# kazuto1011/dusty-gan

Hardware: AMD Instinct MI355X
Metric: G+D train images/sec on 64x1024 LiDAR (steps/sec beside it) (higher is better)
Workload: dtype bf16

## Files before the change

dusty_gan_amd/_lib.py:

```python
import ctypes as C
import os
import subprocess

_HERE = os.path.dirname(os.path.abspath(__file__))
CSRC = os.path.join(_HERE, "csrc")
LIB_PATH = os.path.join(CSRC, "libdustygan_hip.so")
if os.environ.get("DUSTY_GAN_LIB_DIAG"):
    _d = os.environ["DUSTY_GAN_LIB_DIAG"]
    LIB_PATH = os.path.join(CSRC, "libdustygan_hip_diag%s.so" % ("" if _d == "1" else _d))

DG_OK, DG_EINVAL, DG_EUNSUPPORTED, DG_EHIP = 0, 1, 2, 3
DG_F32, DG_BF16 = 0, 1
DG_BF16X2 = 2
MODE_S2, MODE_UP, MODE_GEMM = 0, 1, 2
EPI_LINEAR, EPI_LRELU, EPI_MASK = 0, 1, 2
DG_FORCE_FP32X3 = 0x100
POLICY_BITS = {"brightness": 1, "saturation": 2, "contrast": 4, "translation": 8, "cutout": 16}

_ERR = {1: "DG_EINVAL (bad argument)", 2: "DG_EUNSUPPORTED (shape not supported by the requested kernel)",
        3: "DG_EHIP (HIP runtime error)"}


class DgError(RuntimeError):
    pass
# ... 36 lines not shown
                ("eps", C.c_float), ("ilo", C.c_int), ("ihi", C.c_int), ("n", C.c_long), ("out", C.c_void_p),
                ("out_bf16", C.c_void_p), ("B", C.c_int), ("H", C.c_int), ("W", C.c_int), ("uf", C.c_void_p),
                ("qi", C.c_void_p)]


class DgWgrad(C.Structure):
    _fields_ = [
        ("wmode", C.c_int), ("ring", C.c_int),
        ("B", C.c_int), ("Hc", C.c_int), ("Wc", C.c_int),
        ("Ci", C.c_int), ("Co", C.c_int),
        ("a", C.c_void_p), ("a_sb", C.c_long), ("a_sp", C.c_long), ("a_sc", C.c_long),
        ("g", C.c_void_p), ("g_sb", C.c_long), ("g_sp", C.c_long), ("g_sc", C.c_long),
        ("dw", C.c_void_p), ("scale", C.c_float), ("rowscale", C.c_void_p),
        ("a_dtype", C.c_int), ("g_dtype", C.c_int),
        ("ws", C.c_void_p), ("g_mod", C.c_int),
    ]


XSUM_PARTS = 8


class DgFetch(C.Structure):
    _fields_ = [("pol", C.c_void_p), ("mask", C.c_void_p), ("pool_ctr", C.c_void_p), ("npool", C.c_int),
                ("min_depth", C.c_float), ("max_depth", C.c_float), ("drop_const", C.c_float), ("B", C.c_int), ("HW", C.c_long),
                ("out", C.c_void_p), ("parts", C.c_void_p)]


class DgAugSet(C.Structure):
    _fields_ = [("x", C.c_void_p), ("xsum", C.c_void_p), ("xsum_parts", C.c_int), ("u_b", C.c_void_p), ("u_c", C.c_void_p), ("t_h", C.c_void_p),
                ("t_w", C.c_void_p), ("o_x", C.c_void_p), ("o_y", C.c_void_p)]


class DgOptSeg(C.Structure):
    _fields_ = [("off", C.c_longlong), ("numel", C.c_longlong), ("part", C.c_void_p), ("splits", C.c_int), ("accumulate", C.c_int),
                ("kind", C.c_int), ("ci", C.c_int), ("co", C.c_int), ("shadow_t", C.c_void_p), ("ws_src", C.c_void_p),
                ("ws_coef", C.c_void_p), ("ws_stride", C.c_longlong), ("ws_n", C.c_int), ("ws_bf16", C.c_int),
                ("ws_scale", C.c_float), ("first_block", C.c_int)]


OPT_MAX_SEG = 20


class DgWgradPlan(C.Structure):
    _fields_ = [("variant", C.c_int), ("splits", C.c_int), ("ws_floats", C.c_long), ("tap_pairs", C.c_int)]


class DgWgradReduce(C.Structure):
    _fields_ = [("ws", C.c_void_p), ("dw", C.c_void_p), ("numel", C.c_long), ("splits", C.c_int), ("accumulate", C.c_int)]


class DgConvPlan(C.Structure):
    _fields_ = [("family", C.c_int), ("bm", C.c_int), ("bn", C.c_int), ("tiles", C.c_int), ("workgroups", C.c_int),
                ("tiles_per_wg", C.c_int), ("thin_mfma", C.c_int), ("mask_bits", C.c_int), ("dbias_rows", C.c_int),
                ("sum_parts", C.c_int)]


_P, _I, _L, _F, _D, _U64 = C.c_void_p, C.c_int, C.c_long, C.c_float, C.c_double, C.c_uint64

PROTOTYPES = {
    "dg_conv": [C.POINTER(DgConv), _I, _P],
    "dg_conv_ex": [C.POINTER(DgConv), _I, _I, _P],
    "dg_conv_plan": [C.POINTER(DgConv), _I, _I, C.POINTER(DgConvPlan)],
    "dg_conv_mfma_supported": [C.POINTER(DgConv)],
    "dg_conv_kernel_choice": [C.POINTER(DgConv)],
    "dg_wgrad": [C.POINTER(DgWgrad), _I, _I, _P],
    "dg_wgrad_plan": [C.POINTER(DgWgrad), _I, _I, C.POINTER(DgWgradPlan)],
    "dg_wgrad_group": [C.POINTER(DgWgrad), _I, _I, _I, _P],
    "dg_wgrad_group_plan": [C.POINTER(DgWgrad), _I, _I, _I, C.POINTER(DgWgradPlan)],
    "dg_wgrad_reduce": [C.POINTER(DgWgradReduce), _I, _P],
    "dg_wgrad_mfma_supported": [C.POINTER(DgWgrad)],
    "dg_wgrad_kernel_choice": [C.POINTER(DgWgrad)],
    "dg_wgrad_kernel_variant": [C.POINTER(DgWgrad), _I],
    "dg_wgrad_has_sample_map": [C.POINTER(DgWgrad), _I],
    "dg_blur_fwd": [_P, _P, _I, _I, _I, _I, _I, _P],
    "dg_blur_fwd_mean": [_P, _P, _I, _I, _I, _I, _I, _P, _I, _P, _P],
    "dg_blur_bwd": [_P, _I, _P, _I, _I, _I, _I, _P],
    "dg_blur_bwd_r1": [_P, _I, _P, _F, _P, _I, _I, _I, _I, _P],
    "dg_blur_r1_tangent": [_P, _I, _P, _F, _P, _P, _I, _I, _I, _I, _I, _P],
    "dg_final_fwd": [_P, _I, _P, _P, _F, _I, _L, _P, _P],
    "dg_final_fwd_acc": [_P, _I, _P, _P, _F, _I, _L, _P, _P],
    "dg_final_bwd_data": [_P, _I, _P, _P, _P, _F, _I, _L, _I, _P, _P, _P],
    "dg_batch_wsum": [_P, _I, _P, _F, _I, _L, _P, _P],
    "dg_head_post_fwd": [_P, _P, _P, _I, _I, _F, _F, _I, _L, _P, _P, _P],
    "dg_head_post_fwd_sum": [_P, _P, _P, _I, _I, _F, _F, _I, _L, _P, _P, _P, _P],
    "dg_head_post_bwd": [_P, _P, _P, _P, _P, _I, _F, _F, _I, _L, _F, _F, _P, _P, _P, _I, _P, _P],
    "dg_logistic_noise": [_P, _P, _F, _L, _P, _P],
    "dg_diffaug_fwd": [_P, _P, _P, _P, _P, _P, _P, _I, _I, _I, _I, _P, _P, _P],
    "dg_diffaug_bwd": [_P, _P, _P, _P, _P, _P, _P, _I, _I, _I, _I, _P, _P, _P],
    "dg_diffaug_fwd_acc": [_P, _P, _P, _P, _P, _P, _P, _I, _I, _I, _I, _P, _P, _P],
    "dg_diffaug_fwd_pre": [_P, _P, _P, _P, _P, _P, _P, _I, _I, _I, _I, _P, _P, _P],
    "dg_diffaug_bwd_acc": [_P, _P, _P, _P, _P, _P, _P, _I, _I, _I, _I, _P, _P, _P],
    "dg_diffaug_blur_fwd": [C.POINTER(DgAugSet), _I, _I, _I, _I, _I, _I, _P, _I, _P],
    "dg_blur_bwd_augsum": [_P, _I, _P, _P, _P, _P, _I, _P, _I, _I, _I, _I, _P],
    "dg_diffaug_bwd_pre": [_P, _P, _P, _P, _P, _P, _P, _I, _I, _I, _I, _P, _P, _P],
    "dg_head_post_bwd_aug": [_P, _P, _P, _P, _P, _P, _P, _P, _P, _P, _P, _I, _P, _I, _F, _F, _I, _I, _I, _F, _F, _P, _P, _P,
                             _I, _P, _P],
    "dg_fetch_reals_pool_sum": [_P, _P, _P, _I, _F, _F, _F, _I, _L, _P, _P, _P],
    "dg_nsgan_d": [_P, _P, _I, _F, _P, _P, _P, _P],
    "dg_nsgan_g": [_P, _I, _F, _P, _P, _P],
    "dg_nsgan_d_step": [_P, _P, _I, _F, _P, _P, _P, _P, _P, _P],
    "dg_nsgan_g_step": [_P, _I, _F, _P, _P, _P],
    "dg_gan_d_step": [_I, _F, _P, _P, _I, _F, _P, _P, _P, _P, _P, _P],
    "dg_gan_g_step": [_I, _P, _P, _I, _F, _P, _P, _P],
    "dg_final_gan_bwd": [_I, _I, _F, _P, _P, _I, _F, _I, _P, _P, _P, _P, _P, _P, _I, _P, _F, _L, _I, _P, _P, _P, _P, _P],
    "dg_det_arena": [_P, _L, _P],
    "dg_mean_acc": [_P, _I, _P, _P],
    "dg_fetch_reals": [_P, _P, _F, _F, _F, _L, _P, _P],
# ... 329 lines not shown
```

dusty_gan_amd/csrc/conv_mfma_pp.hip:

```cpp
#include "conv_mfma_persist_impl.h"

#include <type_traits>

namespace pp {

using persist::Geo;
using persist::Tile;

typedef __attribute__((ext_vector_type(4))) float f32x4_t;

#define PP_WAIT(vm) asm volatile("s_waitcnt vmcnt(%0) lgkmcnt(0)" ::"n"(vm) : "memory")

constexpr int NHT = 256;
struct HTab { unsigned long long e[NHT]; };

__device__ __forceinline__ unsigned long long pp_stamp() {
  unsigned long long t;
  __builtin_amdgcn_sched_barrier(0);
  asm volatile("s_memtime %0\n\ts_waitcnt lgkmcnt(0)" : "=s"(t)::"memory");
  __builtin_amdgcn_sched_barrier(0);
  return t;
}

template <int CTRL>
__device__ __forceinline__ float row_add(float v) {
  const int s = __builtin_amdgcn_update_dpp(0, __builtin_bit_cast(int, v), CTRL, 0xf, 0xf, false);
  return v + __builtin_bit_cast(float, s);
}

template <int BN, int MODE, bool MASK, bool DUAL = false, bool BITS = false, bool X2 = false>
__global__ __launch_bounds__(512, 2) void conv_pp_kernel(ConvP p, Geo g, HTab ht) {
  static_assert(MASK || !BITS, "BITS: a flavour of the EPI_MASK epilogue");
  static_assert(!X2 || !BITS, "X2: mask source = the saved activation's hi half");
  static_assert(!DUAL || (MODE == MODE_UP && BN == 128), "DUAL: both column parities of a 64-channel MODE_UP layer");
  constexpr int NCH = DUAL ? BN / 2 : BN;
  constexpr int BM = 256, NWV = 8, WN = 2;
  constexpr int SB = 128;
  constexpr int WC = BN / WN;
  constexpr int TM = 4, TN = WC / 16;
  constexpr int CPL = 4 * TN;
  constexpr int IMG_ROWS = 264;
  constexpr int AIMG = IMG_ROWS * SB;
  constexpr int BT = BN * SB;
  constexpr int PSTAGE = AIMG + 2 * BT;
  constexpr int NPS = 2;
  constexpr int IA = 4, IB = BN / 8 / NWV;
  constexpr int NST = TM * CPL * 2 / 16;
  constexpr int NDB = 512;
  constexpr int NPAIR = MODE == MODE_S2 ? 2 : 1;
  constexpr bool STRIP = BN == 128 && !X2;
  constexpr int SCR = STRIP ? 16 * WC * 2 : 0;
  constexpr int NDBR = 4;
  constexpr int NDBX = MASK ? (NDBR - 2) * NDB : 0;
  constexpr int DBW = DUAL ? NWV : NWV / WN;
  constexpr int LDS_HT = NPS * PSTAGE + 3 * NDB * 4 + NDBX * 4 + NWV * SCR;
  static_assert(IB >= 1 && LDS_HT <= 160 * 1024, "LDS");
  __shared__ __attribute__((aligned(1024))) unsigned char lds[LDS_HT];
#ifdef DG_PP_DIAG
  constexpr int dbg = DG_PP_DIAG;
#else
  constexpr int dbg = 0;
#endif

  const int G = gridDim.x;
  const int q8 = G >> 3, r8 = G & 7, xcd = blockIdx.x & 7;
  const int gi0 = xcd < r8 ? xcd * (q8 + 1) : r8 * (q8 + 1) + (xcd - r8) * q8;
  const int nwx = q8 + (xcd < r8 ? 1 : 0);
// ... 2 lines not shown
  const int xe = (gi0 + nwx) * tq + (gi0 + nwx < tr ? gi0 + nwx : tr);
  const int t0 = xs + (int)(blockIdx.x >> 3);
  const int tcount = t0 < xe ? (xe - t0 + nwx - 1) / nwx : 0;
  if (tcount == 0) {
    if (MASK && p.dbias && p.dbias_part)
      for (int n = threadIdx.x; n < p.N; n += 64 * NWV) p.dbias_part[(long)blockIdx.x * p.N + n] = 0.f;
    return;
  }

  const unsigned long long tk0 = (dbg & 8) ? pp_stamp() : 0ull;
  const unsigned long long tr0 = (dbg & 8) ? __builtin_amdgcn_s_memrealtime() : 0ull;
  const int tid = threadIdx.x;
  const int wave = __builtin_amdgcn_readfirstlane(tid >> 6), lane = tid & 63;
  const int KC = p.K / 64;
  const int Ws = MODE == MODE_S2 ? 2 * p.Wc : p.Wc, cmul = MODE == MODE_S2 ? 2 : 1;
  const int Wo = MODE == MODE_S2 ? p.Wc : 2 * p.Wc;
  const int rows = MODE == MODE_S2 ? p.Hc : 2 * p.Hc;
  const int tiles_n = g.tiles_n, tiles_x = g.tiles_x;

  auto tile_at = [&](int t) {
    Tile r;
    int mt = t / tiles_n;
    r.nt = t % tiles_n;
    r.px = 0;
    r.xt = mt % tiles_x; mt /= tiles_x;
    if (MODE == MODE_UP && !DUAL) { r.px = mt & 1; mt >>= 1; }
    r.Y = mt % rows; r.bt = mt / rows;
    r.nt = __builtin_amdgcn_readfirstlane(r.nt); r.xt = __builtin_amdgcn_readfirstlane(r.xt);
    r.px = __builtin_amdgcn_readfirstlane(r.px); r.Y = __builtin_amdgcn_readfirstlane(r.Y);
    r.bt = __builtin_amdgcn_readfirstlane(r.bt);
    return r;
  };
  const Tile first = tile_at(t0);
  Tile dstep;
  {
    int r = nwx;
    dstep.nt = r % tiles_n; r /= tiles_n;
    dstep.xt = r % tiles_x; r /= tiles_x;
    dstep.px = 0;
    if (MODE == MODE_UP && !DUAL) { dstep.px = r & 1; r >>= 1; }
    dstep.Y = r % rows; dstep.bt = r / rows;
    dstep.nt = __builtin_amdgcn_readfirstlane(dstep.nt); dstep.xt = __builtin_amdgcn_readfirstlane(dstep.xt);
    dstep.px = __builtin_amdgcn_readfirstlane(dstep.px); dstep.Y = __builtin_amdgcn_readfirstlane(dstep.Y);
    dstep.bt = __builtin_amdgcn_readfirstlane(dstep.bt);
  }
  auto tile_next = [&](Tile& t) __attribute__((always_inline)) {
    int c;
    t.nt += dstep.nt; c = t.nt >= tiles_n; if (c) t.nt -= tiles_n;
    t.xt += dstep.xt + c; c = t.xt >= tiles_x; if (c) t.xt -= tiles_x;
    if (MODE == MODE_UP && !DUAL) { t.px += dstep.px + c; c = t.px >> 1; t.px &= 1; }
    t.Y += dstep.Y + c; c = t.Y >= rows; if (c) t.Y -= rows;
    t.bt += dstep.bt + c;
  };

  const bf16* in = (const bf16*)p.in;
  const bf16* w = (const bf16*)p.w;
  const int lrow = lane >> 3, pos = lane & 7;
  auto swzA = [](int row) { return ((row >> 1) & 3) << 1; };
  auto swzB = [](int row) { return ((row >> 1) & 1) | (((row / CPL) & 3) << 1); };

  unsigned voffA[NPAIR][IA + 1], voffB[IB];
  int colA[IA + 1];
  unsigned sampA[IA + 1];
  {
    const int pitch = g.SW + (DUAL ? 2 : 1);
#pragma unroll
    for (int u = 0; u <= IA; ++u) {
      const int m = (u < IA ? (wave + NWV * u) : 32) * 8 + lrow;
      int seg = m / pitch, c = m - seg * pitch;
      if (seg >= g.NSB) { seg = 0; c = 0; }
      colA[u] = cmul * c;
      sampA[u] = (unsigned)(seg * (int)p.in_sb * 2 + (pos ^ swzA(m)) * 16);
    }
  }
#pragma unroll
  for (int u = 0; u < IB; ++u) {
    const int row = (wave + NWV * u) * 8 + lrow;
    voffB[u] = (unsigned)((DUAL ? row & 63 : row) * (int)p.w_sn * 2 + (pos ^ swzB(row)) * 16);
  }
  const unsigned dst_wave = (unsigned)wave * 1024u;

  const int wm = wave >> 1, wn = wave & 1;
  const int a16 = lane & 15, g4 = lane >> 4;
  const unsigned lds0 = (unsigned)(size_t)(__attribute__((address_space(3))) unsigned char*)lds;
  unsigned pbase[2];
  {
    const int rowbase = ((wm * 64) >> g.lsw) * (g.SW + (DUAL ? 2 : 1)) + ((wm * 64) & (g.SW - 1));
#pragma unroll
    for (int t = 0; t < 2; ++t) {
      const int r = rowbase + a16 + t + (DUAL ? wn : 0);
      pbase[t] = (unsigned)(r * SB + ((g4 ^ swzA(r)) << 4));
    }
  }
  const unsigned wrow = (unsigned)(wn * WC + (a16 >> 2) * CPL + (a16 & 3));
  const unsigned wbase = (unsigned)(AIMG + wrow * SB + ((g4 ^ (((a16 >> 1) & 1) | ((a16 >> 2) << 1))) << 4));

  float* s_rs = (float*)(lds + NPS * PSTAGE);
  float* s_bias = s_rs + NDB;
  float* s_db = s_bias + NDB;
  const unsigned srs0 = lds0 + NPS * PSTAGE, sbias0 = srs0 + NDB * 4, sdb0 = sbias0 + NDB * 4;
  const bool want_db = MASK && p.dbias != nullptr;
  const bool db_rows = MASK && DBW * p.N <= NDBR * NDB;
  const unsigned sdbw0 = db_rows ? sbias0 + (unsigned)((DUAL ? wave : wave / WN) * p.N) * 4u : sdb0;
  for (int i = tid; i < NDB; i += 64 * NWV) {
    s_bias[i] = (!MASK && p.bias && i < p.N) ? p.bias[i % p.bias_mod] * (p.epi == EPI_LRELU ? SQRT2 : 1.f) : 0.f;
    s_db[i] = 0.f;
    s_rs[i] = (p.rowscale && i < p.B) ? p.rowscale[i] : 1.f;
  }
  if (MASK)
    for (int i = tid; i < NDBX; i += 64 * NWV) s_db[NDB + i] = 0.f;
  __syncthreads();
  const unsigned long long tk1 = (dbg & 8) ? pp_stamp() : 0ull;

  f32x4_t acc[TM][TN];
  auto zero_acc = [&]() __attribute__((always_inline)) {
#pragma unroll
    for (int i = 0; i < TM; ++i)
#pragma unroll
      for (int j = 0; j < TN; ++j) acc[i][j] = f32x4_t{0.f, 0.f, 0.f, 0.f};
  };
  zero_acc();
  i32x4 fp[2][TM], fw[2][TN];

  bf16* out = (bf16*)p.out;
  const unsigned lane_c0 = (unsigned)((DUAL ? 0 : wn * WC) + g4 * CPL);
  const unsigned lane_coff = X2 ? lane_c0 * 2 + ((lane_c0 >> 6) << 7) : lane_c0 * 2;
  const unsigned par_off = DUAL ? (unsigned)(wn * (int)p.out_sp * 2) : 0u;
  const long px_b = (long)(MODE == MODE_S2 ? 1 : 2) * p.out_sp * 2;
  unsigned pix_off;
  {
    const int trow = wm * 64 + a16;
    const int sb = trow >> g.lsw, x = trow & (g.SW - 1);
    pix_off = (unsigned)((sb * (int)p.out_sb + (MODE == MODE_S2 ? x : 2 * x) * (int)p.out_sp) * 2) + lane_coff + par_off;
  }
  constexpr int CH = WC / 8;
  constexpr int RPB = 64 / CH;
  constexpr int NRD = 16 / RPB;
  static_assert(NRD == NST / TM, "strip geometry");
  auto swzS = [](int px) { return CH == 8 ? (px & 7) : ((px >> 1) & 3); };
  const unsigned scr0 = lds0 + NPS * PSTAGE + 3 * NDB * 4 + NDBX * 4 + (unsigned)wave * SCR;
  const unsigned scr_w = scr0 + (unsigned)(a16 * (CH * 16) + (((g4 * NRD) ^ swzS(a16)) << 4));
  unsigned scr_r, st_off;
  {
    const int pr = lane / CH, c = lane % CH;
    scr_r = scr0 + (unsigned)(pr * (CH * 16) + ((c ^ swzS(pr)) << 4));
    const int trow = wm * 64 + pr;
    const int sb = trow >> g.lsw, x = trow & (g.SW - 1);
    st_off = (unsigned)((sb * (int)p.out_sb + (MODE == MODE_S2 ? x : 2 * x) * (int)p.out_sp) * 2 + c * 16) +
             (DUAL ? par_off : (unsigned)((wn * WC) * 2));
  }
  static_assert(NRD == 1 || RPB * CH * 16 == 1024, "strip read offset");
  auto tile_off = [&](const Tile& t) __attribute__((always_inline)) -> long {
    const int n0 = t.xt * BM;
    return (long)(t.bt * g.NSB) * p.out_sb + ((long)t.Y * Wo + (MODE == MODE_S2 ? n0 : 2 * n0 + t.px)) * p.out_sp +
           t.nt * NCH * (X2 ? 2 : 1);
  };
  i32x4 axr[(MASK && !BITS) ? NST : 1];
  unsigned mbits[BITS ? TM : 1];
  const unsigned pix_off_m = pix_off >> 4;
  auto load_aux = [&](const Tile& t) __attribute__((always_inline)) {
    if constexpr (BITS) {
      const char* mb = (const char*)p.mask_in + (tile_off(t) >> 3);
#pragma unroll
      for (int i = 0; i < TM; ++i) {
        const char* src = mb + (long)i * px_b;
        if (CPL == 16) asm volatile("global_load_ushort %0, %1, %2" : "=v"(mbits[i]) : "v"(pix_off_m), "s"(src) : "memory");
        else asm volatile("global_load_ubyte %0, %1, %2" : "=v"(mbits[i]) : "v"(pix_off_m), "s"(src) : "memory");
      }
    } else {
      const char* ab = (const char*)((const bf16*)p.aux + tile_off(t));
#pragma unroll
      for (int i = 0; i < TM; ++i) {
        const char* src = ab + (long)(i * 16) * px_b;
        asm volatile("global_load_dwordx4 %0, %1, %2" : "=v"(axr[(NST / TM) * i]) : "v"(pix_off), "s"(src) : "memory");
        if (NST / TM == 2) asm volatile("global_load_dwordx4 %0, %1, %2 offset:16" : "=v"(axr[2 * i + 1]) : "v"(pix_off), "s"(src) : "memory");
      }
    }
  };
  auto flush_db = [&](float (&dbacc)[CPL], int nt) __attribute__((always_inline)) {
#pragma unroll
    for (int c = 0; c < CPL; ++c) dbacc[c] = row_add<0xB1>(dbacc[c]);
#pragma unroll
    for (int c = 0; c < CPL; ++c) dbacc[c] = row_add<0x4E>(dbacc[c]);
#pragma unroll
    for (int c = 0; c < CPL; ++c) dbacc[c] = row_add<0x124>(dbacc[c]);
#pragma unroll
    for (int c = 0; c < CPL; ++c) dbacc[c] = row_add<0x128>(dbacc[c]);
    if (a16 == 0) {
      const unsigned ad = sdbw0 + (unsigned)(nt * NCH * 4) + lane_c0 * 4;
#pragma unroll
      for (int c = 0; c < CPL; ++c) asm volatile("ds_add_f32 %0, %1 offset:%2" ::"v"(ad), "v"(dbacc[c]), "n"(c * 4) : "memory");
    }
  };
  auto epilogue = [&](const Tile& t) __attribute__((always_inline)) {
    char* ob = (char*)(out + tile_off(t));
    if (MASK && !BITS) {
#pragma unroll
      for (int i = 0; i < NST; ++i) asm volatile("" : "+v"(axr[i]));
    }
    if (BITS) {
#pragma unroll
      for (int i = 0; i < TM; ++i) asm volatile("" : "+v"(mbits[i]));
    }
    char* mob = nullptr;
    if (!MASK && p.mask_out) mob = (char*)p.mask_out + (tile_off(t) >> 3);
    f32x4_t bias[TN];
    float rs = 0.f;
    if (want_db) {
      const unsigned ra = srs0 + (unsigned)(t.bt * g.NSB + ((wm * 64) >> g.lsw)) * 4;
      asm volatile("ds_read_b32 %0, %1" : "=v"(rs) : "v"(ra) : "memory");
    }
    if (!MASK) {
      const unsigned ba = sbias0 + (unsigned)(t.nt * NCH * 4) + lane_c0 * 4;
#pragma unroll
      for (int j = 0; j < TN; ++j)
        asm volatile("ds_read_b128 %0, %1 offset:%2" : "=v"(bias[j]) : "v"(ba), "n"(j * 16) : "memory");
      asm volatile("s_waitcnt lgkmcnt(0)" ::: "memory");
#pragma unroll
      for (int j = 0; j < TN; ++j) asm volatile("" : "+v"(bias[j]));
    } else {
      asm volatile("s_waitcnt lgkmcnt(0)" ::: "memory");
      asm volatile("" : "+v"(rs));
    }
    float dbacc[CPL];
#pragma unroll
    for (int c = 0; c < CPL; ++c) dbacc[c] = 0.f;
    float c_pos = p.scale * SQRT2, c_neg = p.scale * (LRELU_SLOPE * SQRT2);
    asm volatile("" : "+v"(c_pos), "+v"(c_neg));
    const float c_lin = p.epi == EPI_LRELU ? c_pos : p.scale;
    const float slope = p.epi == EPI_LRELU ? LRELU_SLOPE : 1.f;
    i32x4 rd[NRD];
    unsigned mrow = 0;
    auto store_row = [&](int i) __attribute__((always_inline)) {
      asm volatile("s_waitcnt lgkmcnt(0)" ::: "memory");
#pragma unroll
      for (int h = 0; h < NRD; ++h) {
        asm volatile("" : "+v"(rd[h]));
        char* dstp = ob + (long)(i * 16 + h * RPB) * px_b + st_off;
        if (!(dbg & 128)) *(i32x4*)dstp = rd[h]; else asm volatile("" ::"v"(rd[h]));
      }
// ... 24 lines not shown
              v = acc[i][j][r] * (posv ? c_pos : c_neg);
              dbacc[c] = fmaf(v, rs, dbacc[c]);
            } else {
              v = fmaf(acc[i][j][r], c_lin, bias[j][r]);
              v = fmaxf(v, slope * v);
            }
            v2[q] = v;
          }
          unsigned pw;
          asm("v_cvt_pk_bf16_f32 %0, %1, %2" : "=v"(pw) : "v"(v2[0]), "v"(v2[1]));
          pk[e2] = (int)pw;
          if constexpr (X2) {
            const float l0 = v2[0] - __builtin_bit_cast(float, pw << 16);
            const float l1 = v2[1] - __builtin_bit_cast(float, pw & 0xffff0000u);
            unsigned pl;
            asm("v_cvt_pk_bf16_f32 %0, %1, %2" : "=v"(pl) : "v"(l0), "v"(l1));
            pkl[e2] = (int)pl;
          }
        }
        if (!MASK && mob) {
          unsigned tb[4];
#pragma unroll
          for (int e2 = 0; e2 < 4; ++e2)
            asm("v_pk_max_i16 %0, %1, 0\n\tv_pk_min_u16 %0, %0, 1 op_sel_hi:[1,0]" : "=&v"(tb[e2]) : "v"(pk[e2]));
          const unsigned mm = tb[0] | (tb[1] << 2) | (tb[2] << 4) | (tb[3] << 6);
          const unsigned gb = (mm & 0x55u) | ((mm >> 15) & 0xAAu);
          if (h == 0) mrow = gb; else mrow |= gb << 8;
          if (h == NST / TM - 1) {
            char* dstm = mob + (long)i * px_b;
            if (CPL == 16) asm volatile("global_store_short %0, %1, %2" ::"v"(pix_off_m), "v"(mrow), "s"(dstm) : "memory");
            else asm volatile("global_store_byte %0, %1, %2" ::"v"(pix_off_m), "v"(mrow), "s"(dstm) : "memory");
          }
        }
        if (!STRIP) {
          char* dstp = ob + (long)(i * 16) * px_b + pix_off + h * 16;
          if (!(dbg & 128)) *(i32x4*)dstp = pk; else asm volatile("" ::"v"(pk));
          if constexpr (X2) {
            if (!(dbg & 128)) *(i32x4*)(dstp + 128) = pkl; else asm volatile("" ::"v"(pkl));
          }
          continue;
        }
        if (h == 0 && i > 0) store_row(i - 1);
        asm volatile("ds_write_b128 %0, %1" ::"v"(scr_w ^ (unsigned)(h << 4)), "v"(pk) : "memory");
      }
      if (STRIP) {
        asm volatile("s_waitcnt lgkmcnt(0)" ::: "memory");
#pragma unroll
        for (int h = 0; h < NRD; ++h)
          asm volatile("ds_read_b128 %0, %1 offset:%2" : "=v"(rd[h]) : "v"(scr_r), "n"(h * 1024) : "memory");
      }
      __builtin_amdgcn_sched_barrier(0);
    }
    if (STRIP) store_row(TM - 1);
    if (want_db) flush_db(dbacc, t.nt);
    zero_acc();
  };

  const bool stamps = (dbg & 8) != 0;
  unsigned long long tsum[6] = {0, 0, 0, 0, 0, 0};
  unsigned long long tend = 0, tkf = 0;

  if (wave >= 4) __builtin_amdgcn_s_barrier();
  unsigned so_c = PSTAGE, so_i = 0;
  bool pending = false;
  bool warm = true;
  Tile tprev = first;
  const long tap_b = (long)p.w_st * 2;
  const unsigned spb = (unsigned)p.in_sp * 2u;

  auto dma_s = [&](unsigned voff, const char* sbase, unsigned ldsbase, auto off_tag) __attribute__((always_inline)) {
    constexpr int OFF = decltype(off_tag)::value;
    asm volatile("s_add_u32 m0, %0, %3\n\ts_nop 0\n\tglobal_load_lds_dwordx4 %1, %2"
                 ::"s"(ldsbase), "v"(voff), "s"(sbase), "n"(OFF) : "memory", "scc");
  };

  auto pair_iter = [&](auto iss_tag, const bool first, const int pi, const char* sA, const char* sB0, const char* sB1,
                       const char* sB0b, const char* sB1b) __attribute__((always_inline)) {
    constexpr bool ISS = decltype(iss_tag)::value;
    const bool comp = !warm;
    auto step = [&](auto t_tag) __attribute__((always_inline)) {
      constexpr int t = decltype(t_tag)::value;
      unsigned long long t0 = 0, t1 = 0, t2 = 0, t3 = 0, t4 = 0, t5 = 0;
      if (stamps) { t0 = pp_stamp(); if (tend) tsum[5] += t0 - tend; }
      const bool last = t == 1 && first && !warm;
      {
        const unsigned so = lds0 + so_c;
        const unsigned pa0 = so + pbase[t], pa1 = so + (pbase[t] ^ 64u);
        const unsigned wa0 = so + wbase + t * BT, wa1 = so + ((wbase ^ 64u) + t * BT);
        const unsigned dst = lds0 + so_i + dst_wave;
        constexpr int NP = t == 0 ? IA + IB : IB;
        auto piece = [&](auto q_tag) __attribute__((always_inline)) {
          constexpr int q = decltype(q_tag)::value;
          if (!ISS || (dbg & 1)) return;
          if constexpr (t == 0 && q < IA) dma_s(voffA[pi][q], sA, dst, std::integral_constant<int, NWV * q * 1024>{});
          else if constexpr (t == 0) dma_s(voffB[q - IA], (DUAL && q - IA == 1) ? sB0b : sB0, dst, std::integral_constant<int, AIMG + NWV * (q - IA) * 1024>{});
          else dma_s(voffB[q], (DUAL && q == 1) ? sB1b : sB1, dst, std::integral_constant<int, AIMG + BT + NWV * q * 1024>{});
        };
        if (ISS && t == 0 && wave == 0 && !(dbg & 1))
          dma_s(voffA[pi][IA], sA, lds0 + so_i, std::integral_constant<int, 32 * 1024>{});
        constexpr int NR = 2 * TM + 2 * TN;
        int q = 0;
        auto pieces_upto = [&](int r) __attribute__((always_inline)) {
#define PP_PIECE(Q) if constexpr (Q < NP) { if (q == Q && r * NP >= Q * NR) { piece(std::integral_constant<int, Q>{}); ++q; } }
          PP_PIECE(0) PP_PIECE(1) PP_PIECE(2) PP_PIECE(3) PP_PIECE(4) PP_PIECE(5) PP_PIECE(6) PP_PIECE(7)
#undef PP_PIECE
        };
#pragma unroll
        for (int r = 0; r < NR; ++r) {
          pieces_upto(r);
          if (dbg & 16) continue;
          if (r < 2 * TM) {
            const int i = r >> 1;
            if (r & 1) LDS_READ128(fp[1][i], pa1, i * 16 * SB); else LDS_READ128(fp[0][i], pa0, i * 16 * SB);
// ... 15 lines not shown
#pragma unroll
          for (int i = 0; i < TM; ++i)
#pragma unroll
            for (int jj = 0; jj < TN; ++jj) asm volatile("" ::"v"(acc[i][jj]));
          zero_acc();
        }
        pending = false;
      };
      if (t == 0 && pending && wave >= 4) finish_tile();
      if (stamps) t2 = pp_stamp();
      __builtin_amdgcn_s_barrier();
      if (stamps) t3 = pp_stamp();
      __builtin_amdgcn_sched_barrier(0);
      if (t == 0 && pending) finish_tile();
      __builtin_amdgcn_sched_barrier(0);
      if (comp) {
        if (stamps && tkf == 0) tkf = t3;
#pragma unroll
        for (int ks = 0; ks < 2; ++ks) {
          if (!(dbg & 2)) {
#pragma unroll
            for (int i = 0; i < TM; ++i)
#pragma unroll
              for (int jj = 0; jj < TN; ++jj)
                acc[i][jj] = __builtin_amdgcn_mfma_f32_16x16x32_bf16(__builtin_bit_cast(bf16x8, fw[ks][jj]),
                                                                      __builtin_bit_cast(bf16x8, fp[ks][i]), acc[i][jj], 0, 0, 0);
          }
          if (ks == 0) {
            __builtin_amdgcn_sched_barrier(0);
            if (MASK && last && !(dbg & (4 | 64))) load_aux(tprev);
          }
        }
        if (last) pending = true;
      }
      __builtin_amdgcn_sched_barrier(0);
      if (stamps) t4 = pp_stamp();
      if (ISS || t == 0 || wave < 4) __builtin_amdgcn_s_barrier();
      if (stamps) {
        t5 = pp_stamp();
        tsum[0] += t1 - t0; tsum[1] += t2 - t1; tsum[2] += t3 - t2; tsum[3] += t4 - t3; tsum[4] += t5 - t4;
        tend = t5;
      }
    };
    step(std::integral_constant<int, 0>{});
    step(std::integral_constant<int, 1>{});
    const unsigned sw_ = so_c; so_c = so_i; so_i = sw_;
  };

  Tile ti = first;
  for (int c = 0; c < tcount; ++c) {
    unsigned long long hl;
    int nh;
    {
      const unsigned long long e = ht.e[ti.Y];
      nh = (int)(e >> 60) & 7;
      hl = e & 0x0fffffffffffffffull;
    }
    const char* in_t = (const char*)(in + (long)(ti.bt * g.NSB) * p.in_sb);
    const char* w_t = (const char*)(w + (long)(ti.nt * NCH) * p.w_sn);
    const int x0 = cmul * ti.xt * BM;
#pragma unroll
    for (int pi = 0; pi < NPAIR; ++pi) {
      const int cb = MODE == MODE_S2 ? pi - 1 : ((DUAL || ti.px == 0) ? -1 : 0);
#pragma unroll
      for (int u = 0; u <= IA; ++u)
        voffA[pi][u] = __umul24((unsigned)((x0 + colA[u] + cb) & (Ws - 1)), spb) + sampA[u];
    }
    const int kxa = MODE == MODE_S2 ? 0 : (ti.px == 0 ? 3 : 2), kxb = MODE == MODE_S2 ? 2 : (ti.px == 0 ? 1 : 0);
    bool firstg = true;
    for (int h = 0; h < nh; ++h) {
      const int it_r = (int)(hl & 1023) >> 2, it_ky = (int)hl & 3;
      hl >>= 10;
      const char* sA_row = in_t + (long)it_r * Ws * spb;
      const char* sB_row = w_t + (long)(it_ky * 4) * tap_b;
      for (int kc = 0; kc < (X2 ? 3 : 1) * KC; ++kc) {
        const int kq = X2 ? kc / 3 : kc, sub = X2 ? kc - 3 * kq : 0;
        const char* sA_k = sA_row + kq * (X2 ? 2 * SB : SB) + (sub == 1 ? SB : 0);
        const char* sB_k = sB_row + kq * (X2 ? 2 * SB : SB) + (sub == 2 ? SB : 0);
#pragma unroll
        for (int pi = 0; pi < NPAIR; ++pi) {
          pair_iter(std::true_type{}, firstg, pi, sA_k, sB_k + (long)(kxa + pi) * tap_b, sB_k + (long)(kxb + pi) * tap_b,
                    sB_k + 2 * tap_b, sB_k);
          if (firstg) { firstg = false; warm = false; }
        }
      }
    }
    tprev = ti;
    tile_next(ti);
  }
  pair_iter(std::false_type{}, true, 0, nullptr, nullptr, nullptr, nullptr, nullptr);
  const unsigned long long tk2 = (dbg & 8) ? pp_stamp() : 0ull;
  const unsigned long long tr2 = (dbg & 8) ? __builtin_amdgcn_s_memrealtime() : 0ull;
  if (pending && !(dbg & 4)) {
    asm volatile("s_waitcnt vmcnt(0)" ::: "memory");
    epilogue(tprev);
  }
  if (stamps && blockIdx.x == 0 && lane == 0) {
    float* sink = (float*)p.out + wave * 8;
    asm volatile("s_waitcnt vmcnt(0)" ::: "memory");
    const unsigned long long tk3 = pp_stamp();
    for (int k = 0; k < 6; ++k) sink[k] = (float)tsum[k];
    float* ph = (float*)p.out + 64 + wave * 8;
    ph[0] = (float)(tk1 - tk0); ph[1] = (float)(tkf - tk0); ph[2] = (float)(tk2 - tk0); ph[3] = (float)(tk3 - tk0);
    ph[4] = (float)tcount;
    ph[5] = (float)(tr2 - tr0);
  }
  if (want_db) {
    asm volatile("s_waitcnt vmcnt(0) lgkmcnt(0)" ::: "memory");
    __syncthreads();
    for (int n = tid; n < p.N; n += 64 * NWV) {
      float v;
      if (db_rows) {
        v = s_bias[n];
#pragma unroll
        for (int r = 1; r < DBW; ++r) v += s_bias[r * p.N + n];
      } else v = s_db[n];
      if (p.dbias_part) p.dbias_part[(long)blockIdx.x * p.N + n] = v;
      else atomicAdd(&p.dbias[n % p.bias_mod], v);
    }
  }
}

template <int BN, int MODE, bool MASK, bool DUAL = false, bool X2 = false>
int launch(const ConvP* p, const Geo& g0, hipStream_t stream, int wg_cap, DgConvPlan* plan) {
  constexpr int CPL_ = (BN / 2 / 16) * 4;
  const bool bits_ok = !X2 && p->out_sn == 1 && p->out_sb % 8 == 0 && p->out_sp % CPL_ == 0 && p->N % CPL_ == 0;
  if (!MASK && p->mask_out && !bits_ok) return DG_EUNSUPPORTED;
  const bool bits = MASK && p->mask_in && bits_ok;
  Geo g = g0;
  static int resident = 0;
  if (!resident) {
    int dev = 0, cus = 0;
    HIP_CHECK_RET(hipGetDevice(&dev));
    HIP_CHECK_RET(hipDeviceGetAttribute(&cus, hipDeviceAttributeMultiprocessorCount, dev));
    resident = cus;
  }
  g.dbg = 0;
  const int cap = (wg_cap > 0 && wg_cap < resident) ? wg_cap : resident;
  const int G = g.ntiles < cap ? g.ntiles : cap;
  if (plan) {
    plan->family = 5; plan->bm = DUAL ? 512 : 256; plan->bn = DUAL ? BN / 2 : BN; plan->tiles = g.ntiles; plan->workgroups = G;
    plan->tiles_per_wg = (g.ntiles + G - 1) / G;
    plan->mask_bits = MASK ? (bits ? 2 : 0) : 1;
    plan->dbias_rows = (MASK && (DUAL ? 8 : 4) * p->N <= 2048) ? G : 0;
    return DG_OK;
  }
  HTab ht;
  {
    const int rows = MODE == MODE_S2 ? p->Hc : 2 * p->Hc;
    for (int y = 0; y < NHT; ++y) {
      unsigned long long hl = 0;
      const int nh = y < rows ? persist::pack_htaps<MODE>(p->adj, y, p->Hc, hl) : 0;
      ht.e[y] = hl | ((unsigned long long)nh << 60);
    }
  }
  if constexpr (X2) {
    conv_pp_kernel<BN, MODE, MASK, DUAL, false, true><<<(unsigned)G, 512, 0, stream>>>(*p, g, ht);
  } else if constexpr (MASK) {
    if (bits) conv_pp_kernel<BN, MODE, true, DUAL, true><<<(unsigned)G, 512, 0, stream>>>(*p, g, ht);
    else conv_pp_kernel<BN, MODE, true, DUAL, false><<<(unsigned)G, 512, 0, stream>>>(*p, g, ht);
  } else conv_pp_kernel<BN, MODE, false, DUAL><<<(unsigned)G, 512, 0, stream>>>(*p, g, ht);
  HIP_CHECK_RET(hipGetLastError());
  return DG_OK;
}

}

int dg_conv_mfma_pp_launch(const ConvP* p0, hipStream_t stream, int min_tiles, int wg_cap, DgConvPlan* plan, int dual) {
  if (p0->mode != MODE_S2 && p0->mode != MODE_UP) return DG_EUNSUPPORTED;
  const bool x2 = p0->in_dtype == DG_BF16X2;
  if (p0->in_dtype != p0->out_dtype || p0->in_dtype != p0->w_dtype || (p0->in_dtype != DG_BF16 && !x2)) return DG_EUNSUPPORTED;
  ConvP q = *p0;
  if (x2) {
    if (p0->K % 64 || p0->N % 64 || p0->in_sp % 64 || p0->in_sb % 64 || p0->out_sp % 64 || p0->out_sb % 64 || p0->w_sn % 64 ||
        p0->w_st % 64 || (((size_t)p0->in | (size_t)p0->out | (size_t)p0->w | (size_t)p0->aux) & 255))
      return DG_EUNSUPPORTED;
    if (p0->mask_out || p0->mask_in) return DG_EUNSUPPORTED;
    q.in_sb *= 2; q.in_sp *= 2; q.out_sb *= 2; q.out_sp *= 2; q.w_st *= 2; q.w_sn *= 2;
  }
  const ConvP* p = &q;
  if (p->K % 64 != 0 || !p->ring || p->nscale) return DG_EUNSUPPORTED;
  if (p->mode == MODE_UP && p->adj && p->K < 128) return DG_EUNSUPPORTED;
  if (p->in_sk != 1 || p->w_sk != 1 || p->out_sn != 1) return DG_EUNSUPPORTED;
  if (p->out_sp % 8 != 0 || p->in_sp % 8 != 0 || p->w_sn % 8 != 0) return DG_EUNSUPPORTED;
  if (p->N > 512 || (p->bias && p->bias_mod < p->N && p->N % p->bias_mod != 0)) return DG_EUNSUPPORTED;
  if (p->dbias && p->bias_mod < p->N) return DG_EUNSUPPORTED;
  const int Ws = p->mode == MODE_S2 ? 2 * p->Wc : p->Wc;
  if ((Ws & (Ws - 1)) != 0 || p->in_sp * 2 >= (1 << 24)) return DG_EUNSUPPORTED;
  if ((p->mode == MODE_S2 ? p->Hc : 2 * p->Hc) > 256) return DG_EUNSUPPORTED;
  const bool mask = p->epi == EPI_MASK;
  if (mask ? p->bias != nullptr : p->dbias != nullptr) return DG_EUNSUPPORTED;
  if (p->rowscale && p->B > 512) return DG_EUNSUPPORTED;
  persist::Geo g;
  int bn = 0;
  if (dual && p->mode == MODE_UP && p->N % 128 != 0 && p->N % 64 == 0 && persist::make_geo<256, 64>(p, g) && g.SW >= 64 &&
      g.NSB * (g.SW + 2) <= 264 && g.ntiles / 2 >= min_tiles) {
    g.ntiles /= 2;
    if (x2) return mask ? pp::launch<128, MODE_UP, true, true, true>(p, g, stream, wg_cap, plan)
                        : pp::launch<128, MODE_UP, false, true, true>(p, g, stream, wg_cap, plan);
    return mask ? pp::launch<128, MODE_UP, true, true>(p, g, stream, wg_cap, plan)
                : pp::launch<128, MODE_UP, false, true>(p, g, stream, wg_cap, plan);
  }
  if (p->N % 128 == 0 && persist::make_geo<256, 128>(p, g) && g.SW >= 64 && g.ntiles >= min_tiles) bn = 128;
  else if (p->N % 64 == 0 && persist::make_geo<256, 64>(p, g) && g.SW >= 64 && g.ntiles >= min_tiles) bn = 64;
  if (!bn) return DG_EUNSUPPORTED;
  const int sel = (bn == 128 ? 0 : 4) + (p->mode == MODE_UP ? 2 : 0) + (mask ? 1 : 0);
  if (x2) switch (sel) {
// ... 21 lines not shown
```

include/dusty_gan_hip.h:

```cpp
#ifndef DUSTY_GAN_HIP_H
#define DUSTY_GAN_HIP_H
#include <stdint.h>

#ifdef __cplusplus
extern "C" {
#endif

#define DG_OK 0
#define DG_EINVAL 1
#define DG_EUNSUPPORTED 2
#define DG_EHIP 3

#define DG_F32 0
#define DG_BF16 1
#define DG_BF16X2 2

#define DG_MODE_S2 0
#define DG_MODE_UP 1
#define DG_MODE_GEMM 2

#define DG_EPI_LINEAR 0
#define DG_EPI_LRELU 1
#define DG_EPI_MASK 2

// ... 5 lines not shown
  long in_sb, in_sp, in_sk;
  void* out;
  long out_sb, out_sp, out_sn;
  const void* w;
  long w_st, w_sk, w_sn;
  float scale;
  int epi;
  const float* bias;
  int bias_mod;
  const void* aux;
  float* dbias;
  const float* rowscale;
  int in_dtype, out_dtype, w_dtype;
  const float* nscale;
  const void* up_frag;
  float* dbias_ws;
  float* dbias_part;
  void* mask_out;
  const void* mask_in;
  float* tanh_sum_parts;
} DgConv;
#define DG_UP_FRAG_BYTES (3 * 18 * 1024)
#define DG_DBIAS_SLOTS 32
#define DG_DBIAS_SLOT_FLOATS 1024

typedef struct DgWgrad {
  int wmode, ring;
  int B, Hc, Wc;
  int Ci, Co;
  const void* a;
  long a_sb, a_sp, a_sc;
  const void* g;
  long g_sb, g_sp, g_sc;
  float* dw;
  float scale;
  const float* rowscale;
  int a_dtype, g_dtype;
  float* ws;
  int g_mod;
} DgWgrad;

int dg_conv(const DgConv* p, int force, void* stream);
#define DG_FORCE_FP32X3 0x100
typedef struct DgConvPlan {
  int family;
  int bm, bn;
  int tiles;
  int workgroups;
  int tiles_per_wg;
  int thin_mfma;
  int mask_bits;
  int dbias_rows;
  int sum_parts;
} DgConvPlan;
int dg_conv_ex(const DgConv* p, int force, int wg_cap, void* stream);
int dg_conv_plan(const DgConv* p, int force, int wg_cap, DgConvPlan* plan);
int dg_conv_mfma_supported(const DgConv* p);
int dg_conv_kernel_choice(const DgConv* p);

int dg_wgrad(const DgWgrad* p, int accumulate, int force, void* stream);
typedef struct DgWgradPlan {
  int variant;
  int splits;
  long ws_floats;
  int tap_pairs;
} DgWgradPlan;
int dg_wgrad_plan(const DgWgrad* p, int accumulate, int force, DgWgradPlan* plan);
int dg_wgrad_group(const DgWgrad* items, int n, int force, int rounds, void* stream);
int dg_wgrad_group_plan(const DgWgrad* items, int n, int force, int rounds, DgWgradPlan* plans);
typedef struct DgWgradReduce {
  const float* ws;
  float* dw;
  long numel;
  int splits;
  int accumulate;
} DgWgradReduce;
int dg_wgrad_reduce(const DgWgradReduce* items, int n, void* stream);
int dg_wgrad_mfma_supported(const DgWgrad* p);
int dg_wgrad_kernel_choice(const DgWgrad* p);
int dg_wgrad_kernel_variant(const DgWgrad* p, int force);
int dg_wgrad_has_sample_map(const DgWgrad* p, int force);

int dg_blur_fwd(const float* x, void* out, int dtype, int B, int H, int W, int ring, void* stream);
int dg_blur_fwd_mean(const float* x, void* out, int dtype, int B, int H, int W, int ring, const float* mean_src, int mean_n,
                     float* mean_acc, void* stream);
int dg_blur_bwd(const void* d, int dtype, float* dx, int B, int H, int W, int ring, void* stream);
int dg_blur_bwd_r1(const void* d, int dtype, float* dx, float oscale, float* ssq, int B, int H, int W, int ring, void* stream);
int dg_blur_r1_tangent(const void* d, int dtype, void* out, float oscale, float* ssq, float* mean_acc, int mean_n, int B, int H,
                       int W, int ring, void* stream);

int dg_final_fwd(const void* d4, int dtype, const float* wf, const float* bias, float scale, int B, long n, float* y,
                 void* stream);
int dg_final_fwd_acc(const void* d4, int dtype, const float* wf, const float* bias, float scale, int B, long n, float* y,
                 void* stream);
int dg_final_bwd_data(const void* d4, int dtype, const float* wf, const float* up, const float* rowscale, float scale,
                      int B, long n, int C, void* dd4, float* dbias, void* stream);
int dg_batch_wsum(const void* src, int dtype, const float* coef, float scale, int B, long n, float* out, void* stream);

int dg_head_post_fwd(float* gout, const float* noise_pixel, const float* noise_image, int arch, int training,
                     float tau, float drop_const, int B, long HW, float* mask, float* depth, void* stream);
int dg_head_post_fwd_sum(float* gout, const float* noise_pixel, const float* noise_image, int arch, int training,
                         float tau, float drop_const, int B, long HW, float* mask, float* depth, float* dsum, void* stream);
int dg_head_post_bwd(const float* gout, const float* noise_pixel, const float* noise_image, const float* mask,
                     const float* ddepth, int arch, float tau, float drop_const, int B, long HW, float s_depth,
                     float s_conf, float* draw, float* dbias, void* draw_pm , int cp,
                     float* bias_ws, void* stream);
// ... 185 lines not shown
```

Baseline: 13520.

## Balance persistent conv tiles by XOR-flipping output rows per batch slice

Adds a host-side chooser that simulates per-workgroup load, weighting each output row by its number of vertical taps, and picks a batch-bit shift whose XOR on the row index minimises the worst workgroup load in the persistent conv kernel. Edge rows in the up/stride modes have fewer taps, so remapping which rows each workgroup gets is meant to even out the tail. Because remapping breaks the per-workgroup bias-gradient row ownership, bias partials are written per tile to a scratch buffer and reduced by whichever workgroup finishes a bucket last, using atomic counters. This adds a global scratch allocation, atomics and an extra reduction pass, and the stamp debug path now writes into the output buffer.

```diff
diff --git a/dusty_gan_amd/_lib.py b/dusty_gan_amd/_lib.py
--- a/dusty_gan_amd/_lib.py
+++ b/dusty_gan_amd/_lib.py
@@ -112,7 +112,7 @@
 class DgConvPlan(C.Structure):
     _fields_ = [("family", C.c_int), ("bm", C.c_int), ("bn", C.c_int), ("tiles", C.c_int), ("workgroups", C.c_int),
                 ("tiles_per_wg", C.c_int), ("thin_mfma", C.c_int), ("mask_bits", C.c_int), ("dbias_rows", C.c_int),
-                ("sum_parts", C.c_int)]
+                ("sum_parts", C.c_int), ("row_flip", C.c_int)]
 
 
 _P, _I, _L, _F, _D, _U64 = C.c_void_p, C.c_int, C.c_long, C.c_float, C.c_double, C.c_uint64
diff --git a/dusty_gan_amd/csrc/conv_mfma_pp.hip b/dusty_gan_amd/csrc/conv_mfma_pp.hip
--- a/dusty_gan_amd/csrc/conv_mfma_pp.hip
+++ b/dusty_gan_amd/csrc/conv_mfma_pp.hip
@@ -12,7 +12,7 @@
 #define PP_WAIT(vm) asm volatile("s_waitcnt vmcnt(%0) lgkmcnt(0)" ::"n"(vm) : "memory")
 
 constexpr int NHT = 256;
-struct HTab { unsigned long long e[NHT]; };
+struct HTab { unsigned long long e[NHT]; int fs, fm; float* dbt; int* dbc; };
 
 __device__ __forceinline__ unsigned long long pp_stamp() {
   unsigned long long t;
@@ -121,6 +121,7 @@
     t.Y += dstep.Y + c; c = t.Y >= rows; if (c) t.Y -= rows;
     t.bt += dstep.bt + c;
   };
+  auto row_of = [&](const Tile& t) __attribute__((always_inline)) { return t.Y ^ ((t.bt >> ht.fs) & ht.fm); };
 
   const bf16* in = (const bf16*)p.in;
   const bf16* w = (const bf16*)p.w;
@@ -221,7 +222,7 @@
   static_assert(NRD == 1 || RPB * CH * 16 == 1024, "strip read offset");
   auto tile_off = [&](const Tile& t) __attribute__((always_inline)) -> long {
     const int n0 = t.xt * BM;
-    return (long)(t.bt * g.NSB) * p.out_sb + ((long)t.Y * Wo + (MODE == MODE_S2 ? n0 : 2 * n0 + t.px)) * p.out_sp +
+    return (long)(t.bt * g.NSB) * p.out_sb + ((long)row_of(t) * Wo + (MODE == MODE_S2 ? n0 : 2 * n0 + t.px)) * p.out_sp +
            t.nt * NCH * (X2 ? 2 : 1);
   };
   i32x4 axr[(MASK && !BITS) ? NST : 1];
@@ -246,7 +247,12 @@
       }
     }
   };
-  auto flush_db = [&](float (&dbacc)[CPL], int nt) __attribute__((always_inline)) {
+  const int NPX = (MODE == MODE_UP && !DUAL) ? 2 : 1;
+  auto tile_index = [&](const Tile& t) __attribute__((always_inline)) {
+    return (((t.bt * rows + row_of(t)) * NPX + t.px) * tiles_x + t.xt) * tiles_n + t.nt;
+  };
+  auto flush_db = [&](float (&dbacc)[CPL], const Tile& t) __attribute__((always_inline)) {
+    const int nt = t.nt;
 #pragma unroll
     for (int c = 0; c < CPL; ++c) dbacc[c] = row_add<0xB1>(dbacc[c]);
 #pragma unroll
@@ -255,6 +261,14 @@
     for (int c = 0; c < CPL; ++c) dbacc[c] = row_add<0x124>(dbacc[c]);
 #pragma unroll
     for (int c = 0; c < CPL; ++c) dbacc[c] = row_add<0x128>(dbacc[c]);
+    if (MASK && ht.dbt) {
+      if (a16 == 0) {
+        float* dst = ht.dbt + ((long)tile_index(t) * DBW + (DUAL ? wave : wm)) * NCH + lane_c0;
+#pragma unroll
+        for (int c = 0; c < CPL; c += 4) *(f32x4_t*)(dst + c) = f32x4_t{dbacc[c], dbacc[c + 1], dbacc[c + 2], dbacc[c + 3]};
+      }
+      return;
+    }
     if (a16 == 0) {
       const unsigned ad = sdbw0 + (unsigned)(nt * NCH * 4) + lane_c0 * 4;
 #pragma unroll
@@ -385,13 +399,14 @@
       __builtin_amdgcn_sched_barrier(0);
     }
     if (STRIP) store_row(TM - 1);
-    if (want_db) flush_db(dbacc, t.nt);
+    if (want_db) flush_db(dbacc, t);
     zero_acc();
   };
 
   const bool stamps = (dbg & 8) != 0;
   unsigned long long tsum[6] = {0, 0, 0, 0, 0, 0};
   unsigned long long tend = 0, tkf = 0;
+  int npairs = 0;
 
   if (wave >= 4) __builtin_amdgcn_s_barrier();
   unsigned so_c = PSTAGE, so_i = 0;
@@ -513,10 +528,11 @@
     unsigned long long hl;
     int nh;
     {
-      const unsigned long long e = ht.e[ti.Y];
+      const unsigned long long e = ht.e[row_of(ti)];
       nh = (int)(e >> 60) & 7;
       hl = e & 0x0fffffffffffffffull;
     }
+    if (stamps) npairs += nh * (X2 ? 3 : 1) * KC * NPAIR;
     const char* in_t = (const char*)(in + (long)(ti.bt * g.NSB) * p.in_sb);
     const char* w_t = (const char*)(w + (long)(ti.nt * NCH) * p.w_sn);
     const int x0 = cmul * ti.xt * BM;
@@ -566,7 +582,65 @@
     ph[4] = (float)tcount;
     ph[5] = (float)(tr2 - tr0);
   }
-  if (want_db) {
+  if (stamps && tid == 0) {
+    float* wb = (float*)p.out + 128 + 4 * blockIdx.x;
+    asm volatile("s_waitcnt vmcnt(0)" ::: "memory");
+    wb[0] = (float)(tk2 - tk0); wb[1] = (float)tcount; wb[2] = (float)npairs; wb[3] = (float)(tr2 - tr0);
+  }
+  if (want_db && ht.dbt) {
+    __shared__ int s_fin[64];
+    __shared__ int s_nfin;
+    asm volatile("s_waitcnt vmcnt(0) lgkmcnt(0)" ::: "memory");
+    __threadfence();
+    if (tid == 0) s_nfin = 0;
+    __syncthreads();
+    auto owner = [&](int tp, int& cnt, int& tb, int& stride) {
+      int b = 0;
+      for (int x = 0; x < 8; ++x) {
+        const int gx = x < r8 ? x * (q8 + 1) : r8 * (q8 + 1) + (x - r8) * q8;
+        const int nx = q8 + (x < r8 ? 1 : 0);
+        const int sx = gx * tq + (gx < tr ? gx : tr);
+        const int ex = (gx + nx) * tq + (gx + nx < tr ? gx + nx : tr);
+        if (nx > 0 && tp >= sx && tp < ex) {
+          const int j = (tp - sx) % nx;
+          b = x + 8 * j; tb = sx + j; stride = nx; cnt = (ex - tb + nx - 1) / nx;
+        }
+      }
+      return b;
+    };
+    if (tid == 0) {
+      Tile tt = first;
+      for (int c = 0; c < tcount; ++c) {
+        int cnt = 0, tb = 0, stride = 1;
+        const int b = owner(tile_index(tt), cnt, tb, stride);
+        if (__hip_atomic_fetch_add(ht.dbc + b, 1, __ATOMIC_ACQ_REL, __HIP_MEMORY_SCOPE_AGENT) + 1 == cnt && s_nfin < 64)
+          s_fin[s_nfin++] = b;
+        tile_next(tt);
+      }
+    }
+    __syncthreads();
+    __threadfence();
+    for (int f = 0; f < s_nfin; ++f) {
+      const int b = s_fin[f];
+      const int x = b & 7, j = b >> 3;
+      const int gx = x < r8 ? x * (q8 + 1) : r8 * (q8 + 1) + (x - r8) * q8;
+      const int nx = q8 + (x < r8 ? 1 : 0);
+      const int tb = gx * tq + (gx < tr ? gx : tr) + j;
+      const int ex = (gx + nx) * tq + (gx + nx < tr ? gx + nx : tr);
+      for (int n = tid; n < p.N; n += 64 * NWV) {
+        const int nt = n / NCH, cn = n - nt * NCH;
+        float v = 0.f;
+        for (int r = 0; r < DBW; ++r) {
+          float a = 0.f;
+          for (int t = tb; t < ex; t += nx)
+            if (t % tiles_n == nt) a += ht.dbt[((long)t * DBW + r) * NCH + cn];
+          v = r == 0 ? a : v + a;
+        }
+        p.dbias_part[(long)b * p.N + n] = v;
+      }
+      if (tid == 0) __hip_atomic_store(ht.dbc + b, 0, __ATOMIC_RELAXED, __HIP_MEMORY_SCOPE_AGENT);
+    }
+  } else if (want_db) {
     asm volatile("s_waitcnt vmcnt(0) lgkmcnt(0)" ::: "memory");
     __syncthreads();
     for (int n = tid; n < p.N; n += 64 * NWV) {
@@ -580,6 +654,70 @@
       else atomicAdd(&p.dbias[n % p.bias_mod], v);
     }
   }
+}
+
+static int choose_flip(int G, int ntiles, int tiles_n, int tiles_x, int npx, int rows, const int* nh, int kunits, int key) {
+  if (rows & 1) return -1;
+  bool uniform = true;
+  for (int y = 1; y < rows; ++y) uniform = uniform && nh[y] == nh[0];
+  if (uniform) return -1;
+  struct Entry { int k[7]; int fs; };
+  static thread_local Entry cache[32];
+  static thread_local int ncache = 0, next = 0;
+  const int k[7] = {G, ntiles, tiles_n, tiles_x, npx, kunits, key};
+  for (int i = 0; i < ncache; ++i) {
+    bool hit = true;
+    for (int j = 0; j < 7; ++j) hit = hit && cache[i].k[j] == k[j];
+    if (hit) return cache[i].fs;
+  }
+  constexpr int NO = 5;
+  long worst[NO] = {0, 0, 0, 0, 0};
+  const int q8 = G >> 3, r8 = G & 7;
+  const int tq = ntiles / G, tr = ntiles % G;
+  for (int b = 0; b < G; ++b) {
+    const int xcd = b & 7;
+    const int gi0 = xcd < r8 ? xcd * (q8 + 1) : r8 * (q8 + 1) + (xcd - r8) * q8;
+    const int nwx = q8 + (xcd < r8 ? 1 : 0);
+    const int xe = (gi0 + nwx) * tq + (gi0 + nwx < tr ? gi0 + nwx : tr);
+    long load[NO] = {0, 0, 0, 0, 0};
+    for (int t = gi0 * tq + (gi0 < tr ? gi0 : tr) + (b >> 3); t < xe; t += nwx) {
+      int mt = t / tiles_n / tiles_x;
+      if (npx == 2) mt >>= 1;
+      const int Y = mt % rows, bt = mt / rows;
+      load[0] += (long)nh[Y] * kunits + 1;
+      for (int s = 0; s < NO - 1; ++s) load[1 + s] += (long)nh[Y ^ ((bt >> s) & 1)] * kunits + 1;
+    }
+    for (int o = 0; o < NO; ++o) worst[o] = load[o] > worst[o] ? load[o] : worst[o];
+  }
+  int best = 0;
+  for (int o = 1; o < NO; ++o) if (worst[o] < worst[best]) best = o;
+  const int fs = best - 1;
+  if (ncache < 32) ++ncache;
+  cache[next] = Entry{{k[0], k[1], k[2], k[3], k[4], k[5], k[6]}, fs};
+  next = (next + 1) & 31;
+  return fs;
+}
+
+static bool flip_scratch(hipStream_t stream, size_t floats, float** dbt, int** dbc) {
+  constexpr int NCTR = 1024, NDEV = 64;
+  static char* buf[NDEV] = {};
+  static size_t cap[NDEV] = {};
+  int dev = 0;
+  if (hipGetDevice(&dev) != hipSuccess || dev < 0 || dev >= NDEV) return false;
+  if (floats > cap[dev]) {
+    hipStreamCaptureStatus st = hipStreamCaptureStatusNone;
+    if (hipStreamIsCapturing(stream, &st) != hipSuccess || st != hipStreamCaptureStatusNone) return false;
+    size_t want = cap[dev] ? cap[dev] : (size_t)1 << 20;
+    while (want < floats) want *= 2;
+    void* q = nullptr;
+    if (hipMalloc(&q, NCTR * sizeof(int) + want * sizeof(float)) != hipSuccess) return false;
+    if (hipMemset(q, 0, NCTR * sizeof(int)) != hipSuccess || hipDeviceSynchronize() != hipSuccess) return false;
+    buf[dev] = (char*)q;
+    cap[dev] = want;
+  }
+  *dbc = (int*)buf[dev];
+  *dbt = (float*)(buf[dev] + NCTR * sizeof(int));
+  return true;
 }
 
 template <int BN, int MODE, bool MASK, bool DUAL = false, bool X2 = false>
@@ -599,21 +737,38 @@
   g.dbg = 0;
   const int cap = (wg_cap > 0 && wg_cap < resident) ? wg_cap : resident;
   const int G = g.ntiles < cap ? g.ntiles : cap;
+  HTab ht;
+  const int rows = MODE == MODE_S2 ? p->Hc : 2 * p->Hc;
+  int nh[NHT];
+  for (int y = 0; y < NHT; ++y) {
+    unsigned long long hl = 0;
+    nh[y] = y < rows ? persist::pack_htaps<MODE>(p->adj, y, p->Hc, hl) : 0;
+    ht.e[y] = hl | ((unsigned long long)nh[y] << 60);
+  }
+#ifdef DG_PP_NO_FLIP
+  int fs = -1;
+#else
+  int fs = choose_flip(G, g.ntiles, g.tiles_n, g.tiles_x, (MODE == MODE_UP && !DUAL) ? 2 : 1, rows, nh,
+                             (X2 ? 3 : 1) * (p->K / 64) * (MODE == MODE_S2 ? 2 : 1), (MODE << 16) ^ (p->adj << 15) ^ p->Hc);
+#endif
+  ht.dbt = nullptr;
+  ht.dbc = nullptr;
+  const int dbw = DUAL ? 8 : 4, nch = DUAL ? BN / 2 : BN;
+  const bool rows_form = MASK && p->dbias && p->dbias_part && dbw * p->N <= 2048 && (g.ntiles + G - 1) / G <= 64 && G <= 1024;
+  if (fs >= 0 && MASK && p->dbias && !rows_form) fs = -1;
+  if (fs >= 0 && rows_form && !plan) {
+    const size_t need = (size_t)g.ntiles * dbw * nch;
+    if (!flip_scratch(stream, need, &ht.dbt, &ht.dbc)) fs = -1;
+  }
+  ht.fs = fs < 0 ? 0 : fs;
+  ht.fm = fs < 0 ? 0 : 1;
   if (plan) {
     plan->family = 5; plan->bm = DUAL ? 512 : 256; plan->bn = DUAL ? BN / 2 : BN; plan->tiles = g.ntiles; plan->workgroups = G;
     plan->tiles_per_wg = (g.ntiles + G - 1) / G;
     plan->mask_bits = MASK ? (bits ? 2 : 0) : 1;
     plan->dbias_rows = (MASK && (DUAL ? 8 : 4) * p->N <= 2048) ? G : 0;
+    plan->row_flip = fs + 1;
     return DG_OK;
-  }
-  HTab ht;
-  {
-    const int rows = MODE == MODE_S2 ? p->Hc : 2 * p->Hc;
-    for (int y = 0; y < NHT; ++y) {
-      unsigned long long hl = 0;
-      const int nh = y < rows ? persist::pack_htaps<MODE>(p->adj, y, p->Hc, hl) : 0;
-      ht.e[y] = hl | ((unsigned long long)nh << 60);
-    }
   }
   if constexpr (X2) {
     conv_pp_kernel<BN, MODE, MASK, DUAL, false, true><<<(unsigned)G, 512, 0, stream>>>(*p, g, ht);
diff --git a/include/dusty_gan_hip.h b/include/dusty_gan_hip.h
--- a/include/dusty_gan_hip.h
+++ b/include/dusty_gan_hip.h
@@ -81,6 +81,7 @@
   int mask_bits;
   int dbias_rows;
   int sum_parts;
+  int row_flip;
 } DgConvPlan;
 int dg_conv_ex(const DgConv* p, int force, int wg_cap, void* stream);
 int dg_conv_plan(const DgConv* p, int force, int wg_cap, DgConvPlan* plan);
```

After: 11550, median of 6. -14.5%, worse.
